# PASSIONLab/ELBA

Measured on AMD Instinct MI355X. Metric: overlap nnz/sec (A·Aᵀ SpGEMM, SharedSeeds semiring, after Prune(numshared<=1)), higher is better.
Workload: dtype u32

## Files before the change

### elba_amd/csrc/capi.hip

```cpp
#include "common.hpp"
#include <new>

using namespace elba;

struct elba_ctx {
    Ctx c;
};

namespace {

template <class F>
int guarded(elba_ctx *ctx, F &&f)
{
    if (!ctx) return ELBA_ERR_INVALID_ARG;
    try {
        ELBA_HIP(hipSetDevice(ctx->c.device));
        f(ctx->c);
        return ELBA_OK;
    } catch (const Error &e) {
        ctx->c.last_error = e.msg;
        return e.code;
    } catch (const std::bad_alloc &) {
        ctx->c.last_error = "host allocation failed";
        return ELBA_ERR_OUT_OF_MEMORY;
// ... 662 lines not shown
                        v->a_csr_format = c.csr_inline ? ELBA_CSR_INLINE : (c.csr_suffix ? ELBA_CSR_DENSE : (c.csr_hints ? ELBA_CSR_HINTS : ELBA_CSR_PLAIN));
                        v->a_csr_pos_mask = c.csr_suffix ? 0xFFFFu : (c.csr_hints ? 0x3FFFFFFFu : 0xFFFFFFFFu);
                        v->a_kmers = c.A_has_kmers ? c.rel_kmers.p : nullptr;
                        v->a_gather_slots = c.use_ell && c.ell_compact ? c.ell_nslots : 0;
                        v->a_slot_kid = c.use_ell && c.ell_compact ? c.ell_slot_kid.p : nullptr; }
        if (c.have_B) { v->Y = c.Y; v->b_rowptr = c.b_rowptr.p; v->b_col = c.b_col.p; v->b_val = c.b_val.p; }
    });
}

int elba_set_option(elba_ctx *ctx, const char *name, int64_t value)
{
    return guarded(ctx, [&](Ctx &c) {
        ELBA_REQUIRE(name, ELBA_ERR_INVALID_ARG, "set_option: null name");
        struct { const char *n; bool *b; } flags[] = {
            {"overlap_cold_calls", &c.cold_calls}, {"no_symmetry", &c.opt.no_symmetry}, {"no_ell", &c.opt.no_ell}, {"no_pay", &c.opt.no_pay}, {"mir32", &c.opt.mir32},
            {"no_hints", &c.opt.no_hints}, {"no_sample", &c.opt.no_sample}, {"no_slab", &c.opt.no_slab}, {"no_ell_compact", &c.opt.no_ell_compact}, {"msd_no_emit8", &c.opt.msd_no_emit8}, {"msd_no_rank", &c.opt.msd_no_rank}, {"msd_rank", &c.opt.msd_rank}, {"csr_pairs_late", &c.opt.csr_pairs_late}, {"no_suffix", &c.opt.no_suffix}, {"ov_generic", &c.opt.ov_generic}, {"no_row_order", &c.opt.no_row_order}, {"no_inline", &c.opt.no_inline}, {"panel_inline", &c.opt.panel_inline}, {"kmer_pairs", &c.opt.kmer_pairs},
            {"kmer_unfused", &c.opt.kmer_unfused}, {"kmer_no_msd", &c.opt.kmer_no_msd}, {"kmer_msd", &c.opt.kmer_msd}, {"csr_pairs", &c.opt.csr_pairs}, {"emit_plain", &c.opt.emit_plain}, {"trace", &c.opt.trace}, {"measure_prep", &c.opt.measure_prep}};
        for (auto &f : flags) if (!strcmp(name, f.n)) { *f.b = value != 0; return; }
        if (!strcmp(name, "kmer_drop")) { ELBA_REQUIRE(value >= 0 && value <= 3, ELBA_ERR_INVALID_ARG, "set_option: kmer_drop is 0..3"); c.opt.kmer_drop = (int)value; }
        else if (!strcmp(name, "dense_up")) { ELBA_REQUIRE(value >= 0 && value <= 3, ELBA_ERR_INVALID_ARG, "set_option: dense_up is 0..3"); c.opt.dense_up = (int)value; }
        else if (!strcmp(name, "dense_wgs")) { ELBA_REQUIRE(value >= 1 && value <= 16, ELBA_ERR_INVALID_ARG, "set_option: dense_wgs is 1..16"); c.opt.dense_wgs = (int)value; }
        else if (!strncmp(name, "tune", 4) && name[4] >= '0' && name[4] <= '7' && name[5] == 0) c.opt.tune[name[4] - '0'] = value;
        else if (!strcmp(name, "msd_small_cap")) c.opt.msd_small_cap = (int)value;
        else if (!strcmp(name, "kmer_batch_instances")) { ELBA_REQUIRE(value >= 0, ELBA_ERR_INVALID_ARG, "set_option: kmer_batch_instances is >= 0"); c.opt.kmer_batch_instances = value; }
        else if (!strcmp(name, "msd_wide_bits")) c.opt.msd_wide_bits = (int)value;
        else if (!strcmp(name, "ell_slot_cap")) c.opt.ell_slot_cap = (int)value;
        else if (!strcmp(name, "slab_pct")) { ELBA_REQUIRE(value >= 1 && value <= 1000, ELBA_ERR_INVALID_ARG, "set_option: slab_pct is 1..1000"); c.opt.slab_pct = (int)value; }
        else if (!strcmp(name, "slab_q16")) { ELBA_REQUIRE(value >= 0 && value < (1ll << 31), ELBA_ERR_INVALID_ARG, "set_option: slab_q16 is 0..2^31"); c.opt.slab_q16 = (int)value; }
        else if (!strcmp(name, "dk")) { ELBA_REQUIRE(value == -1 || value == 0 || value == 1 || value == 2 || value == 4, ELBA_ERR_INVALID_ARG, "set_option: dk is -1 (chosen per matrix), 0, 1, 2 or 4"); c.opt.dk = (int)value; }
        else if (!strcmp(name, "aln_tiers")) { ELBA_REQUIRE(value >= 0, ELBA_ERR_INVALID_ARG, "set_option: aln_tiers is a string of the digits 1, 2, 4, 8"); c.opt.aln_tiers = value; }
        else if (!strcmp(name, "aln_wide_hint")) c.opt.aln_wide_hint = (int)value;
// ... 21 lines not shown

int elba_get_stat(elba_ctx *ctx, const char *name, int64_t *value)
{
    return guarded(ctx, [&](Ctx &c) {
        ELBA_REQUIRE(name && value, ELBA_ERR_INVALID_ARG, "get_stat: null name or value");
        if (!strcmp(name, "overlap_mirror_placed")) *value = c.ov_mir_placed;
        else if (!strcmp(name, "overlap_slab_q16")) *value = (int64_t)c.ov_slab_q16_used;
        else if (!strcmp(name, "kmer_path")) *value = c.kmer_path;
        else if (!strcmp(name, "kmer_passes")) *value = c.kmer_passes;
        else if (!strcmp(name, "kmer_crowded_buckets")) *value = c.kmer_crowded;
        else if (!strcmp(name, "kmer_crowded_small")) *value = c.kmer_crowded_small;
        else if (!strcmp(name, "kmer_largest_pass")) *value = c.kmer_largest_pass;
        else if (!strcmp(name, "kmer_peak_bytes")) *value = c.kmer_peak_bytes;
        else if (!strcmp(name, "kmer_buckets")) *value = c.kmer_buckets;
        else if (!strcmp(name, "overlap_passes")) *value = c.ov_passes;
        else if (!strcmp(name, "overlap_spec")) *value = c.ov_spec;
        else if (!strcmp(name, "overlap_forwarded")) *value = c.ov_forwarded;
        else if (!strcmp(name, "spgemm_prep_us")) *value = c.prep_us;
        else if (!strcmp(name, "emit_us")) *value = c.emit_us;
        else if (!strcmp(name, "triples_path")) *value = c.triples_path;
        else if (!strcmp(name, "padded_columns")) *value = c.have_A && c.use_ell ? 1 : 0;
        else if (!strcmp(name, "gather_slots")) *value = c.have_A && c.use_ell ? c.ell_nslots : 0;
        else if (!strcmp(name, "contig_count")) *value = c.have_contigs ? c.cstats.contigs : 0;
        else if (!strcmp(name, "contig_cycles")) *value = c.have_contigs ? c.cstats.cycles : 0;
        else if (!strcmp(name, "contig_circular")) *value = c.have_contigs ? c.cg_circular : 0;
        else if (!strcmp(name, "contig_singletons")) *value = c.have_contigs ? c.cg_singletons : 0;
        else if (!strcmp(name, "contig_reads")) *value = c.have_contigs ? c.cstats.contig_reads : 0;
        else if (!strcmp(name, "contig_bases")) *value = c.have_contigs ? c.cstats.bases : 0;
        else if (!strcmp(name, "contig_branches")) *value = c.have_contigs ? c.cstats.branches : 0;
        else if (!strcmp(name, "contig_rank_us")) *value = c.have_contigs ? (int64_t)(c.cstats.ms_rank * 1000.0f) : -1;
// ... 150 lines not shown
```

### elba_amd/csrc/common.hpp

```cpp
#pragma once
#include <hip/hip_runtime.h>
#include <cstdint>
#include <cstdio>
#include <cstdlib>
#include <cstring>
#include <mutex>
#include <string>
#include <vector>
#include "../../include/elba_amd.h"

namespace elba {

struct Error {
    int code;
    std::string msg;
};

#define ELBA_HIP(expr)                                                                                   \
    do {                                                                                                 \
        hipError_t e__ = (expr);                                                                         \
        if (e__ != hipSuccess) {                                                                         \
            throw ::elba::Error{e__ == hipErrorOutOfMemory ? ELBA_ERR_OUT_OF_MEMORY : ELBA_ERR_HIP,      \
                                std::string(#expr) + ": " + hipGetErrorString(e__) + " (" + __FILE__ +  \
                                    ":" + std::to_string(__LINE__) + ")"};                               \
// ... 108 lines not shown
    bool no_hints = false;
    bool no_sample = false;
    bool no_ell_compact = false;
    bool no_slab = false;
    bool csr_pairs_late = false;
    bool msd_rank = false;
    bool msd_no_rank = false;
    bool msd_no_emit8 = false;
    int ell_slot_cap = 0;
    int slab_pct = 175;
    int slab_q16 = 0;
    bool panel_inline = false;
    bool no_inline = false;
    bool no_suffix = false;
    bool ov_generic = false;
    bool no_row_order = false;
    bool kmer_pairs = false;
    bool kmer_unfused = false;
    bool kmer_msd = false;
    bool kmer_no_msd = false;
    bool csr_pairs = false;
    bool emit_plain = false;
    bool trace = false;
    bool measure_prep = false;
    int64_t tune[8] = {0, 0, 0, 0, 0, 0, 0, 0};
    int msd_wide_bits = 0;
    int64_t kmer_batch_instances = 0;
    int msd_small_cap = 0;
    int kmer_drop = 0;
    int dense_up = 1;
// ... 128 lines not shown
    DevBuf ov_rowub, ov_rowcnt, ov_rowoff, ov_lists, ov_counters, ov_gtable, ov_sortkeys;
    int64_t ov_tmp_cap = 0;
    bool ov_sort_used[2] = {false, false};
    bool ov_tiers_known = false, ov_tier_used[8] = {false, false, false, false, false, false, false, false};
    int64_t b_cap_entries = 0;
    uint64_t ov_calls = 0;
    uint32_t ov_prior_q16 = 0;
    uint32_t ov_slab_q16 = 0;
    DevBuf ov_slab;
    int64_t ov_slab_cap = 0;
    DevBuf ov_tickrows;
    DevBuf ov_slabpos, ov_slabn;
    bool ov_slab_on = false;
    uint32_t ov_slab_q16_used = 0;
    int64_t ov_mir_placed = 0;
    int64_t ov_spec = 0;
    int64_t ov_passes = 0, ov_forwarded = 0;
    int ov_phase = 0;
    int ov_pend_passes = 1; bool ov_pend_timed = false; float ov_pend_ms[3] = {0, 0, 0};
    std::vector<uint64_t> ov_remote_bounds;
    DevBuf ov_remote;
    int64_t ov_send_slot = 0;
    DevBuf ov_cursors;
    bool own_stream = true;

    EventTimer t_total, t_a, t_b, t_c;
    EventTimer t_emit, t_emit_plain; int64_t prep_us = -1, emit_us = -1;
    struct PinnedHost { void *p = nullptr; size_t cap = 0; void reserve(size_t n) { if (n <= cap) return; if (p) (void)hipHostFree(p); p = nullptr; cap = 0; ELBA_HIP(hipHostMalloc(&p, n, hipHostMallocDefault)); cap = n; } ~PinnedHost() { if (p) (void)hipHostFree(p); } };
    PinnedHost ov_host;
    PhaseMarks<5> ov_marks;
// ... 50 lines not shown
```

### elba_amd/csrc/spgemm.hip

```cpp
#include "common.hpp"
#include <algorithm>
#include <type_traits>

namespace elba {

namespace {

constexpr uint32_t EMPTY = 0xFFFFFFFFu;
constexpr int NUM_LDS_TIERS = 5;
constexpr int NUM_TIERS = NUM_LDS_TIERS + 1;
constexpr int LDS_TBITS0 = 9;
constexpr uint32_t STAGE_CHUNK = 1024;
constexpr uint32_t FIN_WAVE_MAX = 256;
constexpr uint32_t FIN_WAVE2_MAX = 1024;
constexpr uint32_t FIN_LDS_MAX = 4096;

struct alignas(128) OvShard {
    unsigned long long yraw, nnz, ndiag, nupper, fb_claims, fb_ub, products;
    unsigned int maxshared;
    unsigned int tier_done[NUM_TIERS];
};
constexpr int NUM_SHARDS = 64;

struct OvCounters {
// ... 896 lines not shown
    static DeviceOnce attr_once;
    attr_once.run(c.device, [&] {
        const int lds = 160 * 1024;
#define ELBA_ATTR(B, P, D) ELBA_HIP(hipFuncSetAttribute(reinterpret_cast<const void *>(&k_spgemm_direct<B, false, P, D>), hipFuncAttributeMaxDynamicSharedMemorySize, lds))
        ELBA_HIP(hipFuncSetAttribute(reinterpret_cast<const void *>(&k_spgemm_direct<512, false, false, 2, true>), hipFuncAttributeMaxDynamicSharedMemorySize, lds));
        ELBA_HIP(hipFuncSetAttribute(reinterpret_cast<const void *>(&k_spgemm_direct<1024, false, false, 2, true>), hipFuncAttributeMaxDynamicSharedMemorySize, lds));
        ELBA_HIP(hipFuncSetAttribute(reinterpret_cast<const void *>(&k_spgemm_direct<1024, false, false, 2, true, 11>), hipFuncAttributeMaxDynamicSharedMemorySize, lds));
        ELBA_ATTR(512, true, 0); ELBA_ATTR(1024, true, 0); ELBA_ATTR(256, false, 0); ELBA_ATTR(512, false, 0); ELBA_ATTR(1024, false, 0);
        ELBA_ATTR(512, true, 1); ELBA_ATTR(512, true, 2); ELBA_ATTR(512, true, 4); ELBA_ATTR(1024, true, 1); ELBA_ATTR(1024, true, 2); ELBA_ATTR(1024, true, 4);
        ELBA_ATTR(256, false, 1); ELBA_ATTR(256, false, 2); ELBA_ATTR(256, false, 4);
        ELBA_ATTR(512, false, 1); ELBA_ATTR(512, false, 2); ELBA_ATTR(512, false, 4); ELBA_ATTR(1024, false, 1); ELBA_ATTR(1024, false, 2); ELBA_ATTR(1024, false, 4);
#undef ELBA_ATTR
#define ELBA_ATTR(B) ELBA_HIP(hipFuncSetAttribute(reinterpret_cast<const void *>(&k_spgemm_direct<B, false, false, 0, false, 0, true>), hipFuncAttributeMaxDynamicSharedMemorySize, lds))
        ELBA_ATTR(128); ELBA_ATTR(256); ELBA_ATTR(512); ELBA_ATTR(1024);
#undef ELBA_ATTR
    });

    c.ov_host.reserve(sizeof(OvCounters));
    OvCounters &hc = *static_cast<OvCounters *>(c.ov_host.p);
    hc = OvCounters{};
    uint32_t skipped_tiers = 0, skipped_sorts = 0;
    int passes = 0;
    c.ov_passes = 0; c.ov_forwarded = 0; c.ov_spec = 0;
    float ms_sym = 0, ms_num = 0, ms_fin = 0, ms_tot = 0;
    bool was_timed = true;
    for (;;) {
        ++passes;
        const int stride = c.cfg.timing_stride > 1 ? c.cfg.timing_stride : 1;
        const bool timed = passes > 1 || (c.ov_calls++ % (uint64_t)stride) == 0;
        c.ov_tmp.reserve((size_t)c.ov_tmp_cap * sizeof(StageRec));
        p.tmp = c.ov_tmp.as<StageRec>(); p.tmp_cap = (unsigned long long)c.ov_tmp_cap;
        const bool mir16 = c.pos16 && !c.opt.mir32;
        c.ov_rec16 = mir16;
        p.rec16 = mir16 ? 1u : 0u; p.rec = c.ov_tmp.as<uint4>(); p.tick = reinterpret_cast<uint32_t *>(c.ov_tmp.as<char>() + (size_t)c.ov_tmp_cap * 16);
        c.b_cap_entries = half ? 2 * c.ov_tmp_cap : c.ov_tmp_cap;
        c.b_col.reserve((size_t)(c.b_cap_entries + 1) * 4);
        c.b_val.reserve((size_t)(c.b_cap_entries + 1) * sizeof(elba_seed_t));
        if (half) c.ov_mir.reserve((size_t)(c.b_cap_entries + 1) * (mir16 ? 16 : sizeof(StageRec)));
// ... 39 lines not shown
        if (nrows > 0) {
            auto X = [&](int B, bool P) { return (size_t)256 + (size_t)(B / 64) * (P ? 3072 : (pay16 ? 2048 : 2560)); };
            const bool all_tiers = !c.ov_tiers_known || phase == 2;
            skipped_tiers = 0;
            int tmax = NUM_TIERS;
            if (c.opt.tune[4] != 2 && passes == 1) {
                const uint64_t ubm = std::min<uint64_t>((uint64_t)std::max<int64_t>(c.max_row_nnz, 1) * (uint64_t)p.max_col, (uint64_t)p.Mcols);
                const int gmax = ubm <= 1 ? 1 : 64 - __builtin_clzll(2 * ubm - 1);
                tmax = gmax <= LDS_TBITS0 ? 0 : gmax - LDS_TBITS0;
                tmax = std::max(tmax, (int)p.min_tier);
                if (p.suffix) tmax = std::max(tmax, (int)p.dense_up);
            }
#define ELBA_DTIER(t, stmt) do { if ((all_tiers || c.ov_tier_used[t]) && (t) <= tmax) { stmt; } else skipped_tiers |= 1u << (t); } while (0)
#define ELBA_LAUNCH_D(B, G, P, grid, lds, tier, tb, smp)                                                                                  \
    do {                                                                                                                                  \
        if (spec && !(G) && !(P))                                                                                                         \
            hipLaunchKernelGGL((k_spgemm_direct<B, false, false, 0, false, 0, true>), dim3(grid), dim3(B), (lds), s, ov_spec_params(p), (tier), (tb), (smp)); \
        else if (dk == 0) hipLaunchKernelGGL((k_spgemm_direct<B, G, P, 0>), dim3(grid), dim3(B), (lds), s, p, (tier), (tb), (smp));            \
        else if (dk == 1) hipLaunchKernelGGL((k_spgemm_direct<B, G, P, 1>), dim3(grid), dim3(B), (lds), s, p, (tier), (tb), (smp));       \
        else if (dk == 4) hipLaunchKernelGGL((k_spgemm_direct<B, G, P, 4>), dim3(grid), dim3(B), (lds), s, p, (tier), (tb), (smp));       \
        else hipLaunchKernelGGL((k_spgemm_direct<B, G, P, 2>), dim3(grid), dim3(B), (lds), s, p, (tier), (tb), (smp));                    \
    } while (0)
            const int dk = c.opt.dk >= 0 ? c.opt.dk : ((c.csr_inline && c.N > 0 && c.Z < 3 * c.N) ? 0 : 1);
            const bool spec = ov_spec_ok(c, p, pay, dk);
            c.ov_spec = spec ? 1 : 0;
#define ELBA_LAUNCH_S(B, TBC, grid, lds, tier, tb, smp) hipLaunchKernelGGL((k_spgemm_direct<B, false, false, 2, true, TBC>), dim3((tier) == 0 ? cus * c.opt.dense_wgs : (grid)), dim3(B), (size_t)18 * (1u << (tb)) + 256 + (size_t)((B) / 64) * 2368, s, p, (tier), (tb), (smp))
            if (sampling) {
                if (p.suffix) ELBA_LAUNCH_S(1024, 0, cus, (size_t)26 * 4096 + X(1024, true), 3, 12u, 1u);
                else if (pay) ELBA_LAUNCH_D(1024, false, true, cus, (size_t)26 * 4096 + X(1024, true), 3, 12u, 1u);
                else ELBA_LAUNCH_D(1024, false, false, cus, (size_t)18 * 4096 + X(1024, false), 3, 12u, 1u);
                p.use_feedback = 0;
            }
            {
                int nb = (int)((nrows + 255) / 256);
                if (nb > cus * 4) nb = cus * 4;
                hipLaunchKernelGGL(k_classify_direct, dim3(nb), dim3(256), 0, s, p, 0);
            }
            if (p.suffix) {
                ELBA_DTIER(0, ELBA_LAUNCH_S(256, 9, cus * 9, (size_t)26 * 512 + X(128, true), 0, 9u, 0u));
                if (p.dense_up >= 1u) ELBA_DTIER(1, ELBA_LAUNCH_S(512, 10, cus * 4, (size_t)26 * 1024 + X(256, true), 1, 10u, 0u));
// ... 286 lines not shown
```

### elba_amd/csrc/spgemm_direct.hpp

```cpp

enum : uint32_t { D_NEXT = 20, D_FB0 = 16, W_ACC_P = 54 , W_END2 = 56 };
constexpr uint32_t RING = 128;
constexpr uint32_t NOROW = 0xFFFFFFFFu, UNRESOLVED = 0xFFFFFFFEu;

__device__ __forceinline__ uint32_t wave_max_scan(uint32_t v)
{
    int x = (int)v, t;
    t = __builtin_amdgcn_update_dpp(0, x, 0x111 , 0xf, 0xf, false); x = t > x ? t : x;
    t = __builtin_amdgcn_update_dpp(0, x, 0x112 , 0xf, 0xf, false); x = t > x ? t : x;
    t = __builtin_amdgcn_update_dpp(0, x, 0x114 , 0xf, 0xf, false); x = t > x ? t : x;
    t = __builtin_amdgcn_update_dpp(0, x, 0x118 , 0xf, 0xf, false); x = t > x ? t : x;
    t = __builtin_amdgcn_update_dpp(0, x, 0x142 , 0xa, 0xf, false); x = t > x ? t : x;
    t = __builtin_amdgcn_update_dpp(0, x, 0x143 , 0xc, 0xf, false); x = t > x ? t : x;
    return (uint32_t)x;
}

__device__ __forceinline__ uint32_t wave_sum_dpp(uint32_t v)
{
    int x = (int)v;
    x += __builtin_amdgcn_update_dpp(0, x, 0x111 , 0xf, 0xf, false);
    x += __builtin_amdgcn_update_dpp(0, x, 0x112 , 0xf, 0xf, false);
    x += __builtin_amdgcn_update_dpp(0, x, 0x114 , 0xf, 0xf, false);
    x += __builtin_amdgcn_update_dpp(0, x, 0x118 , 0xf, 0xf, false);
    x += __builtin_amdgcn_update_dpp(0, x, 0x142 , 0xa, 0xf, false);
// ... 6 lines not shown
    int x = (int)v;
    x += __builtin_amdgcn_update_dpp(0, x, 0x111 , 0xf, 0xf, false);
    x += __builtin_amdgcn_update_dpp(0, x, 0x112 , 0xf, 0xf, false);
    x += __builtin_amdgcn_update_dpp(0, x, 0x114 , 0xf, 0xf, false);
    x += __builtin_amdgcn_update_dpp(0, x, 0x118 , 0xf, 0xf, false);
    x += __builtin_amdgcn_update_dpp(0, x, 0x142 , 0xa, 0xf, false);
    x += __builtin_amdgcn_update_dpp(0, x, 0x143 , 0xc, 0xf, false);
    return (uint32_t)x;
}

__device__ __forceinline__ bool owns_pair(uint32_t i, uint32_t j, uint32_t row_lo, uint32_t row_hi, bool upper = false)
{
    return j < row_lo || j >= row_hi || (upper ? j > i : ((((i ^ j) & 1u) != 0u) ? j < i : j > i));
}

template <int BLOCK, bool GLOBAL, bool PAY, int DK = 2, bool SUFFIX = false, int TB = 0, bool SPEC = false>
#ifndef ELBA_DENSE_OCC
#define ELBA_DENSE_OCC 8
#endif
__global__ __launch_bounds__(BLOCK, SUFFIX ? ELBA_DENSE_OCC : (DK == 4 ? 1 : 4)) void k_spgemm_direct(std::conditional_t<SPEC, OvSpecParams, OvParams> p, int tier, uint32_t lds_tbits, uint32_t sample)
{
    static_assert(!PAY || !GLOBAL, "payload accumulators: LDS tiers only");
    static_assert(!SPEC || (!GLOBAL && !PAY && !SUFFIX), "the reads path: LDS tiers, 32-bit accumulators carrying posT");
    extern __shared__ __attribute__((aligned(16))) uint32_t smem[];
    uint32_t *misc = GLOBAL ? smem : smem + (size_t)(PAY ? 6 : 4) * (1u << lds_tbits) + ((size_t)1 << lds_tbits) / 2;
    const uint32_t tid = threadIdx.x, lane = tid & 63;
    const uint64_t lt = (1ull << lane) - 1;
    const uint32_t nrows = sample ? p.ctr->sample_count : p.ctr->tier_count[tier];
    if (nrows == 0) return;
    const uint32_t lb = p.lpc_log2, sub = tid & ((1u << lb) - 1u), grp = tid >> lb, EPT = (uint32_t)BLOCK >> lb;
    const uint32_t fbits = p.fbits, fmask = (1u << fbits) - 1u, stride = p.s_stride;
    const bool ell = SPEC || p.a_ell != nullptr;
    const uint32_t hmask = p.hint_mask, pmask = p.pos_mask;
    const uint2 *csr2 = reinterpret_cast<const uint2 *>(p.a_csr);
    const uint32_t slab_q = (p.slab != nullptr && !sample) ? sfirst(p.ctr->slab_q16) : 0u;
    unsigned long long chunk_off = 0;
// ... 126 lines not shown
            tab.keys[s2] = EMPTY; tab.cnt[s2] = 0;
            if (PAY) { tab.vmin[s2] = ~0ull; tab.vmax[s2] = 0ull; } else { tab.smin[s2] = 0xFFFFFFFFu; tab.smax[s2] = 0; }
        };
        const uint32_t DG = GLOBAL ? 0u : dpar;

        bool full = false;
        uint32_t dg = 0, pr = 0;
        uint32_t head = 0, tail = 0;
        const bool pay16 = !PAY && !SUFFIX && !GLOBAL && p.pay16 != 0u;
        uint32_t *qj = misc + 64 + (tid >> 6) * (SUFFIX ? 592u : (PAY ? 768u : (pay16 ? 512u : 640u)));
        uint32_t *qs = qj + RING;
        unsigned long long *qv = reinterpret_cast<unsigned long long *>(qj + RING);
        auto drain = [&](uint32_t n) {
            const uint32_t at = (head + lane) & (RING - 1u);
            const uint32_t j = qj[at];
            if (PAY) { const unsigned long long v = qv[at]; tab.insert_lds64(j, v, v, 1u, lane < n, full); }
            else { const uint32_t sq = qs[at]; tab.insert_lds(j, sq, sq, 1u, lane < n, full); }
            head += n;
        };
        auto slot = [&](uint32_t j, uint32_t posT, uint32_t seq, uint32_t posQ) {
            const uint64_t mv = __ballot(j != EMPTY);
            if (mv == 0) return;
            const uint64_t md = __ballot(j == i);
            pr += (uint32_t)__popcll(mv); dg += (uint32_t)__popcll(md);
            uint64_t mi = mv & ~md;
            if (p.half) mi &= __ballot(owns_pair(i, j, p.half == 2u ? 0u : p.row_lo, p.half == 2u ? 0xFFFFFFFFu : p.row_hi, !PAY && p.suffix != 0u));
            if (mi == 0) return;
            const bool ins = (mi >> lane) & 1ull;
            if (GLOBAL) { if (ins) tab.insert(j, seq, full); return; }
            const uint32_t at = (tail + (uint32_t)__popcll(mi & lt)) & (RING - 1u);
            if (ins) {
                qj[at] = j;
// ... 264 lines not shown
        uint32_t yraw = 0;
        const bool relabel = SUFFIX && p.row_label != nullptr, whole = p.row_lo == 0u && p.row_hi == p.M;
        if (!GLOBAL && T == 4u * (uint32_t)BLOCK) {
            uint32_t jj[4], cc[4], pre[4], tot = 0;
            uint64_t bal[4];
#pragma unroll
            for (int u = 0; u < 4; ++u) { jj[u] = tab.keys[(uint32_t)u * BLOCK + tid]; cc[u] = tab.cnt[(uint32_t)u * BLOCK + tid]; }
            if (SUFFIX && relabel && !whole) {
#pragma unroll
                for (int u = 0; u < 4; ++u) if (jj[u] != EMPTY) jj[u] = p.row_order[jj[u]];
            }
#pragma unroll
            for (int u = 0; u < 4; ++u) {
                const uint32_t j = jj[u];
                if (j != EMPTY) yraw += (p.half == 2u || (p.half && j >= p.row_lo && j < p.row_hi)) ? 2u : 1u;
                bal[u] = __ballot(j != EMPTY && cc[u] >= 2u);
                if (j != EMPTY && cc[u] < 2u) reset_slot((uint32_t)u * BLOCK + tid);
                pre[u] = tot; tot += (uint32_t)__popcll(bal[u]);
            }
            if (tot) {
                uint32_t at = 0;
                if (lane == 0) asm volatile("ds_add_rtn_u32 %0, %1, %2\n\ts_waitcnt lgkmcnt(0)" : "=v"(at) : "v"((uint32_t)(uintptr_t)&misc[3]), "v"(tot) : "memory");
                at = sfirst(at);
#pragma unroll
                for (int u = 0; u < 4; ++u)
                    if ((bal[u] >> lane) & 1ull) list16[at + pre[u] + (uint32_t)__popcll(bal[u] & lt)] = (uint16_t)((uint32_t)u * BLOCK + tid);
            }
        } else
        for (uint32_t b0 = 0; b0 < T; b0 += BLOCK) {
            const uint32_t s0 = b0 + tid;
            bool keep = false;
            if (s0 < T) {
                uint32_t j = tab.ld(tab.keys, s0);
                if (j != EMPTY) {
                    if (SUFFIX && relabel && !whole) j = p.row_order[j];
                    yraw += (p.half == 2u || (p.half && j >= p.row_lo && j < p.row_hi)) ? 2u : 1u; keep = tab.ld(tab.cnt, s0) >= 2;
                    if (!GLOBAL && !keep) reset_slot(s0);
                }
            }
            const uint64_t bal = __ballot(keep);
            if (bal == 0) continue;
            uint32_t at = 0;
            if (lane == 0) at = atomicAdd(&misc[3], (uint32_t)__popcll(bal));
            at = __shfl(at, 0, 64) + (uint32_t)__popcll(bal & lt);
            if (keep) { if (GLOBAL) list[at] = s0; else list16[at] = (uint16_t)s0; }
        }
        yraw = wave_sum_dpp(yraw);
        if (lane == 0 && yraw) lds_add32(&misc[5], yraw);
        if (GLOBAL) __syncthreads(); else lds_barrier();
        ELBA_DSTAMP(4);
        if (tid == 0) {
// ... 29 lines not shown
            const uint32_t ysurv = ysurv_row;
            const uint32_t hasd = dcount_row >= 2 ? 1u : 0u;
            uint32_t nup = 0, mx = 0, nmir = 0;
            bool drew = false;
            auto seed_at = [&](uint32_t a, uint32_t &q, uint32_t &t) {
                const uint2 ce = csr2[rs + (a >> fbits)];
                if (p.inl != 0u && (ce.y >> 31) != 0u) { q = ce.x & 0xFFFFu; t = ce.x >> 16; return; }
                q = ce.x & pmask;
                t = ell ? (uint32_t)p.a_ell[(unsigned long long)ce.y * stride + (a & fmask)] : (uint32_t)p.a_csc[p.a_colptr[ce.y] + (a & fmask)];
            };
            for (uint32_t t = tid; t < ysurv + hasd; t += BLOCK) {
                elba_seed_t v;
                uint32_t j = i;
                if (t < ysurv) {
                    const uint32_t s0 = GLOBAL ? __hip_atomic_load(&list[t], __ATOMIC_RELAXED, __HIP_MEMORY_SCOPE_AGENT) : (uint32_t)list16[t];
                    j = tab.ld(tab.keys, s0); v.numshared = (int32_t)tab.ld(tab.cnt, s0);
                    if (SUFFIX && relabel) j = p.row_order[j];
                    if (PAY) {
                        const uint32_t va = (uint32_t)tab.vmin[s0], vb = (uint32_t)tab.vmax[s0];
                        v.q0 = va >> 16; v.t0 = va & 0xFFFFu; v.q1 = vb >> 16; v.t1 = vb & 0xFFFFu;
                    } else if (pay16) {
                        const uint32_t va = tab.ld(tab.smin, s0), vb = tab.ld(tab.smax, s0);
                        const uint2 ca2 = csr2[rs + ((va >> 16) >> fbits)], cb2 = csr2[rs + ((vb >> 16) >> fbits)];
                        v.q0 = (p.inl != 0u && (ca2.y >> 31) != 0u) ? (ca2.x & 0xFFFFu) : (ca2.x & pmask); v.t0 = va & 0xFFFFu;
                        v.q1 = (p.inl != 0u && (cb2.y >> 31) != 0u) ? (cb2.x & 0xFFFFu) : (cb2.x & pmask); v.t1 = vb & 0xFFFFu;
                    } else {
                        seed_at(tab.ld(tab.smin, s0), v.q0, v.t0);
                        seed_at(tab.ld(tab.smax, s0), v.q1, v.t1);
                    }
                    if (!GLOBAL) reset_slot(s0);
                } else {
// ... 50 lines not shown
        if (*w64(W_MIR)) atomicAdd(&sh->nnz, *w64(W_MIR));
        if (misc[W_MX]) atomicMax(&sh->maxshared, misc[W_MX]);
        unsigned long long fc = *w64(W_FB_C), fu = *w64(W_FB_U);
        if (p.use_feedback && misc[W_FB_N]) { atomicAdd(&p.ctr->fb_claims, fc); atomicAdd(&p.ctr->fb_ub, fu); }
        if (sample && *w64(W_ACC_Y)) atomicAdd(&p.ctr->fb_surv, *w64(W_ACC_Y));
        fc += *w64(W_TOT_C); fu += *w64(W_TOT_U);
        if (fu) { atomicAdd(&sh->fb_claims, fc); atomicAdd(&sh->fb_ub, fu); }
        if (misc[W_ACC_DONE]) {
            atomicAdd(&sh->yraw, *w64(W_ACC_YRAW));
            atomicAdd(&sh->nnz, *w64(W_ACC_Y));
            atomicAdd(&sh->products, *w64(W_ACC_P));
            atomicAdd(&sh->tier_done[tier], misc[W_ACC_DONE]);
            if (misc[W_ACC_NDIAG]) atomicAdd(&sh->ndiag, (unsigned long long)misc[W_ACC_NDIAG]);
        }
    }
}

__global__ __launch_bounds__(256) void k_classify_direct(OvParams p, int mode)
{
    const uint32_t stride = gridDim.x * blockDim.x;
    const uint32_t lane = threadIdx.x & 63;
    const uint64_t lt = (1ull << lane) - 1;
    if (mode == 1) {
        for (uint32_t q = blockIdx.x * blockDim.x + threadIdx.x; q < p.nsample; q += stride) {
            const uint32_t i = p.row_lo + q * p.sstep;
            if (i < p.row_hi && p.a_rowptr[i + 1] != p.a_rowptr[i]) p.sample_list[atomicAdd(&p.ctr->sample_count, 1u)] = i;
        }
        return;
    }
    uint32_t prior_q16 = p.prior_q16;
// ... 67 lines not shown
```

### elba_amd/csrc/spgemm_table.hpp

```cpp
enum : uint32_t {
    W_ACC_YRAW = 32 , W_ACC_Y = 34 , W_ACC_DONE = 36, W_ACC_NDIAG = 37, W_FB_N = 38,
    W_FB_C = 40 , W_FB_U = 42 , W_TOT_C = 44 , W_TOT_U = 46 , W_NUP = 48 , W_MIR = 50 , W_MX = 52, W_END = 54
};
#if defined(ELBA_HMIX_SEL) && ELBA_HMIX_SEL == 1
#define ELBA_HMIX(j) ((j) ^ ((j) >> 5))
#elif defined(ELBA_HMIX_SEL) && ELBA_HMIX_SEL == 2
#define ELBA_HMIX(j) (((j) * 0x85EBCA6Bu) ^ ((j) >> 3))
#elif defined(ELBA_HMIX_SEL) && ELBA_HMIX_SEL == 3
#define ELBA_HMIX(j) ((j) ^ ((j) << 7))
#else
#define ELBA_HMIX(j) (j)
#endif
template <bool GLOBAL>
struct Table {
    uint32_t *keys, *cnt, *smin, *smax, *misc;
    unsigned long long *vmin, *vmax;
    uint32_t tbits, limit;
    __device__ __forceinline__ uint32_t size() const { return 1u << tbits; }
    __device__ __forceinline__ bool abandoned() const { return !GLOBAL && __hip_atomic_load(&misc[10], __ATOMIC_RELAXED, __HIP_MEMORY_SCOPE_WORKGROUP) != 0; }
    __device__ __forceinline__ void insert(uint32_t j, uint32_t s, bool &full) const
    {
        if (full) return;
        const uint32_t mask = size() - 1;
        uint32_t slot = (ELBA_HMIX(j) * 0x9E3779B1u) >> (32 - tbits);
// ... 47 lines not shown
                : [base] "s"(base), [empty] "v"(empty), [j] "v"(j), [mask] "s"(mask), [tb] "s"(tb), [one] "v"(cnt), [s] "v"(s), [smx] "v"(smx)
                : "vcc", "memory");
        }
        if (__ballot(claimed != 0) != 0) {
            uint32_t prev = 0;
            if (claimed) {
                const uint32_t a9 = (uint32_t)(uintptr_t)&misc[9], one = 1u;
                asm volatile("ds_add_rtn_u32 %0, %1, %2\n\ts_waitcnt lgkmcnt(0)" : "=v"(prev) : "v"(a9), "v"(one) : "memory");
            }
            if (__ballot(claimed != 0 && prev >= limit) != 0) {
                misc[10] = 1u;
                full = true;
            }
        }
    }
    __device__ __forceinline__ void insert_lds64(uint32_t j, unsigned long long lo, unsigned long long hi, uint32_t cnt, bool valid, bool &full) const
    {
        if (full) return;
        uint32_t slot = lds_slot(j);
        uint32_t claimed = 0, old, addr = 0;
        unsigned long long save, t;
        const uint32_t base = (uint32_t)(uintptr_t)keys;
        const uint32_t base64 = (uint32_t)(uintptr_t)vmin;
        const uint32_t mask = size() - 1, empty = EMPTY;
        const uint32_t tb = size() * 4, tb8 = size() * 8;
        if (valid) {
            asm volatile(
                "s_mov_b64 %[save], exec\n"
                ".Lprobe%=:\n\t"
                "v_lshl_add_u32 %[addr], %[slot], 2, %[base]\n\t"
                "ds_cmpst_rtn_b32 %[old], %[addr], %[empty], %[j]\n\t"
                "s_waitcnt lgkmcnt(0)\n\t"
                "v_cmp_eq_u32_e64 %[t], %[old], %[empty]\n\t"
                "v_cndmask_b32_e64 %[cl], %[cl], 1, %[t]\n\t"
                "v_cmp_eq_u32_e32 vcc, %[old], %[j]\n\t"
                "s_or_b64 vcc, vcc, %[t]\n\t"
                "s_andn2_b64 exec, exec, vcc\n\t"
                "s_cbranch_execz .Ldone%=\n\t"
                "v_add_u32_e32 %[slot], 1, %[slot]\n\t"
                "v_and_b32_e32 %[slot], %[mask], %[slot]\n\t"
                "s_branch .Lprobe%=\n"
                ".Ldone%=:\n\t"
                "s_mov_b64 exec, %[save]\n\t"
                "v_add_u32_e32 %[old], %[tb], %[addr]\n\t"
                "ds_add_u32 %[old], %[one]\n\t"
                "v_lshl_add_u32 %[old], %[slot], 3, %[base64]\n\t"
                "ds_min_u64 %[old], %[lo]\n\t"
                "v_add_u32_e32 %[old], %[tb8], %[old]\n\t"
                "ds_max_u64 %[old], %[hi]\n"
                : [save] "=&s"(save), [addr] "+v"(addr), [old] "=&v"(old), [t] "=&s"(t), [cl] "+v"(claimed), [slot] "+v"(slot)
                : [base] "s"(base), [base64] "s"(base64), [empty] "v"(empty), [j] "v"(j), [mask] "s"(mask), [tb] "s"(tb), [tb8] "s"(tb8), [one] "v"(cnt), [lo] "v"(lo), [hi] "v"(hi)
                : "vcc", "memory");
        }
        if (__ballot(claimed != 0) != 0) {
            uint32_t prev = 0;
            if (claimed) {
                const uint32_t a9 = (uint32_t)(uintptr_t)&misc[9], one = 1u;
                asm volatile("ds_add_rtn_u32 %0, %1, %2\n\ts_waitcnt lgkmcnt(0)" : "=v"(prev) : "v"(a9), "v"(one) : "memory");
            }
            if (__ballot(claimed != 0 && prev >= limit) != 0) {
                misc[10] = 1u;
                full = true;
            }
        }
    }
    __device__ __forceinline__ uint32_t hit4_lds(const uint32_t (&j)[4], uint32_t s0) const
    {
        typedef __attribute__((address_space(3))) uint32_t lds_u32;
        const lds_u32 *lk = (const lds_u32 *)keys;
        const uint32_t T = size(), tb = T * 4;
        uint32_t slot[4], k[4], m[4];
#pragma unroll
        for (int r = 0; r < 4; ++r) slot[r] = lds_slot(j[r]);
#pragma unroll
        for (int r = 0; r < 4; ++r) {
            k[r] = __hip_atomic_load(&lk[slot[r]], __ATOMIC_RELAXED, __HIP_MEMORY_SCOPE_WORKGROUP);
            m[r] = __hip_atomic_load(&lk[slot[r] + 2u * T], __ATOMIC_RELAXED, __HIP_MEMORY_SCOPE_WORKGROUP);
        }
        uint32_t miss = 0;
        const uint32_t base = (uint32_t)(uintptr_t)keys, one = 1u;
// ... 110 lines not shown
```

Measured before the change: 16.93 billion.

## Aggregate hash-table claim counting per wavefront and skip count add on claim

```diff
diff --git a/elba_amd/csrc/capi.hip b/elba_amd/csrc/capi.hip
--- a/elba_amd/csrc/capi.hip
+++ b/elba_amd/csrc/capi.hip
@@ -700,7 +700,7 @@
         ELBA_REQUIRE(name, ELBA_ERR_INVALID_ARG, "set_option: null name");
         struct { const char *n; bool *b; } flags[] = {
             {"overlap_cold_calls", &c.cold_calls}, {"no_symmetry", &c.opt.no_symmetry}, {"no_ell", &c.opt.no_ell}, {"no_pay", &c.opt.no_pay}, {"mir32", &c.opt.mir32},
-            {"no_hints", &c.opt.no_hints}, {"no_sample", &c.opt.no_sample}, {"no_slab", &c.opt.no_slab}, {"no_ell_compact", &c.opt.no_ell_compact}, {"msd_no_emit8", &c.opt.msd_no_emit8}, {"msd_no_rank", &c.opt.msd_no_rank}, {"msd_rank", &c.opt.msd_rank}, {"csr_pairs_late", &c.opt.csr_pairs_late}, {"no_suffix", &c.opt.no_suffix}, {"ov_generic", &c.opt.ov_generic}, {"no_row_order", &c.opt.no_row_order}, {"no_inline", &c.opt.no_inline}, {"panel_inline", &c.opt.panel_inline}, {"kmer_pairs", &c.opt.kmer_pairs},
+            {"no_hints", &c.opt.no_hints}, {"no_sample", &c.opt.no_sample}, {"no_slab", &c.opt.no_slab}, {"no_ell_compact", &c.opt.no_ell_compact}, {"msd_no_emit8", &c.opt.msd_no_emit8}, {"msd_no_rank", &c.opt.msd_no_rank}, {"msd_rank", &c.opt.msd_rank}, {"csr_pairs_late", &c.opt.csr_pairs_late}, {"no_suffix", &c.opt.no_suffix}, {"ov_generic", &c.opt.ov_generic}, {"ov_claim_legacy", &c.opt.ov_claim_legacy}, {"no_row_order", &c.opt.no_row_order}, {"no_inline", &c.opt.no_inline}, {"panel_inline", &c.opt.panel_inline}, {"kmer_pairs", &c.opt.kmer_pairs},
             {"kmer_unfused", &c.opt.kmer_unfused}, {"kmer_no_msd", &c.opt.kmer_no_msd}, {"kmer_msd", &c.opt.kmer_msd}, {"csr_pairs", &c.opt.csr_pairs}, {"emit_plain", &c.opt.emit_plain}, {"trace", &c.opt.trace}, {"measure_prep", &c.opt.measure_prep}};
         for (auto &f : flags) if (!strcmp(name, f.n)) { *f.b = value != 0; return; }
         if (!strcmp(name, "kmer_drop")) { ELBA_REQUIRE(value >= 0 && value <= 3, ELBA_ERR_INVALID_ARG, "set_option: kmer_drop is 0..3"); c.opt.kmer_drop = (int)value; }
@@ -752,6 +752,7 @@
         else if (!strcmp(name, "kmer_peak_bytes")) *value = c.kmer_peak_bytes;
         else if (!strcmp(name, "kmer_buckets")) *value = c.kmer_buckets;
         else if (!strcmp(name, "overlap_passes")) *value = c.ov_passes;
+        else if (!strcmp(name, "overlap_claim_insert")) *value = c.ov_claim_insert;
         else if (!strcmp(name, "overlap_spec")) *value = c.ov_spec;
         else if (!strcmp(name, "overlap_forwarded")) *value = c.ov_forwarded;
         else if (!strcmp(name, "spgemm_prep_us")) *value = c.prep_us;
diff --git a/elba_amd/csrc/common.hpp b/elba_amd/csrc/common.hpp
--- a/elba_amd/csrc/common.hpp
+++ b/elba_amd/csrc/common.hpp
@@ -146,6 +146,7 @@
     bool no_inline = false;
     bool no_suffix = false;
     bool ov_generic = false;
+    bool ov_claim_legacy = false;
     bool no_row_order = false;
     bool kmer_pairs = false;
     bool kmer_unfused = false;
@@ -304,6 +305,7 @@
     bool ov_slab_on = false;
     uint32_t ov_slab_q16_used = 0;
     int64_t ov_mir_placed = 0;
+    int64_t ov_claim_insert = 1;
     int64_t ov_spec = 0;
     int64_t ov_passes = 0, ov_forwarded = 0;
     int ov_phase = 0;
diff --git a/elba_amd/csrc/spgemm.hip b/elba_amd/csrc/spgemm.hip
--- a/elba_amd/csrc/spgemm.hip
+++ b/elba_amd/csrc/spgemm.hip
@@ -934,6 +934,9 @@
 #define ELBA_ATTR(B) ELBA_HIP(hipFuncSetAttribute(reinterpret_cast<const void *>(&k_spgemm_direct<B, false, false, 0, false, 0, true>), hipFuncAttributeMaxDynamicSharedMemorySize, lds))
         ELBA_ATTR(128); ELBA_ATTR(256); ELBA_ATTR(512); ELBA_ATTR(1024);
 #undef ELBA_ATTR
+#define ELBA_ATTR(B) ELBA_HIP(hipFuncSetAttribute(reinterpret_cast<const void *>(&k_spgemm_direct_claim0<B>), hipFuncAttributeMaxDynamicSharedMemorySize, lds))
+        ELBA_ATTR(128); ELBA_ATTR(256); ELBA_ATTR(512); ELBA_ATTR(1024);
+#undef ELBA_ATTR
     });
 
     c.ov_host.reserve(sizeof(OvCounters));
@@ -941,7 +944,7 @@
     hc = OvCounters{};
     uint32_t skipped_tiers = 0, skipped_sorts = 0;
     int passes = 0;
-    c.ov_passes = 0; c.ov_forwarded = 0; c.ov_spec = 0;
+    c.ov_passes = 0; c.ov_forwarded = 0; c.ov_spec = 0; c.ov_claim_insert = 1;
     float ms_sym = 0, ms_num = 0, ms_fin = 0, ms_tot = 0;
     bool was_timed = true;
     for (;;) {
@@ -1011,7 +1014,9 @@
 #define ELBA_DTIER(t, stmt) do { if ((all_tiers || c.ov_tier_used[t]) && (t) <= tmax) { stmt; } else skipped_tiers |= 1u << (t); } while (0)
 #define ELBA_LAUNCH_D(B, G, P, grid, lds, tier, tb, smp)                                                                                  \
     do {                                                                                                                                  \
-        if (spec && !(G) && !(P))                                                                                                         \
+        if (spec && !(G) && !(P) && c.opt.ov_claim_legacy)                                                                                \
+            hipLaunchKernelGGL((k_spgemm_direct_claim0<B>), dim3(grid), dim3(B), (lds), s, ov_spec_params(p), (tier), (tb), (smp));       \
+        else if (spec && !(G) && !(P))                                                                                                    \
             hipLaunchKernelGGL((k_spgemm_direct<B, false, false, 0, false, 0, true>), dim3(grid), dim3(B), (lds), s, ov_spec_params(p), (tier), (tb), (smp)); \
         else if (dk == 0) hipLaunchKernelGGL((k_spgemm_direct<B, G, P, 0>), dim3(grid), dim3(B), (lds), s, p, (tier), (tb), (smp));            \
         else if (dk == 1) hipLaunchKernelGGL((k_spgemm_direct<B, G, P, 1>), dim3(grid), dim3(B), (lds), s, p, (tier), (tb), (smp));       \
@@ -1021,6 +1026,7 @@
             const int dk = c.opt.dk >= 0 ? c.opt.dk : ((c.csr_inline && c.N > 0 && c.Z < 3 * c.N) ? 0 : 1);
             const bool spec = ov_spec_ok(c, p, pay, dk);
             c.ov_spec = spec ? 1 : 0;
+            c.ov_claim_insert = spec ? (c.opt.ov_claim_legacy ? 0 : 2) : 1;
 #define ELBA_LAUNCH_S(B, TBC, grid, lds, tier, tb, smp) hipLaunchKernelGGL((k_spgemm_direct<B, false, false, 2, true, TBC>), dim3((tier) == 0 ? cus * c.opt.dense_wgs : (grid)), dim3(B), (size_t)18 * (1u << (tb)) + 256 + (size_t)((B) / 64) * 2368, s, p, (tier), (tb), (smp))
             if (sampling) {
                 if (p.suffix) ELBA_LAUNCH_S(1024, 0, cus, (size_t)26 * 4096 + X(1024, true), 3, 12u, 1u);
diff --git a/elba_amd/csrc/spgemm_direct.hpp b/elba_amd/csrc/spgemm_direct.hpp
--- a/elba_amd/csrc/spgemm_direct.hpp
+++ b/elba_amd/csrc/spgemm_direct.hpp
@@ -44,12 +44,12 @@
     return j < row_lo || j >= row_hi || (upper ? j > i : ((((i ^ j) & 1u) != 0u) ? j < i : j > i));
 }
 
-template <int BLOCK, bool GLOBAL, bool PAY, int DK = 2, bool SUFFIX = false, int TB = 0, bool SPEC = false>
-#ifndef ELBA_DENSE_OCC
-#define ELBA_DENSE_OCC 8
-#endif
-__global__ __launch_bounds__(BLOCK, SUFFIX ? ELBA_DENSE_OCC : (DK == 4 ? 1 : 4)) void k_spgemm_direct(std::conditional_t<SPEC, OvSpecParams, OvParams> p, int tier, uint32_t lds_tbits, uint32_t sample)
+template <int BLOCK, bool GLOBAL, bool PAY, int DK, bool SUFFIX, int TB, bool SPEC, int INS>
+__device__ __forceinline__ void spgemm_direct_rows(std::conditional_t<SPEC, OvSpecParams, OvParams> p, int tier, uint32_t lds_tbits, uint32_t sample)
 {
+    static_assert(INS != 0 || (SPEC && !PAY), "the insert of rounds 1-6: kept for the reads path's A/B only");
+    static_assert(INS == 0 || INS == 1 || (INS == 2 && SPEC), "count - 1 in the count words: the reads path only");
+    constexpr uint32_t CKEEP = INS == 2 ? 1u : 2u, CBIAS = INS == 2 ? 1u : 0u;
     static_assert(!PAY || !GLOBAL, "payload accumulators: LDS tiers only");
     static_assert(!SPEC || (!GLOBAL && !PAY && !SUFFIX), "the reads path: LDS tiers, 32-bit accumulators carrying posT");
     extern __shared__ __attribute__((aligned(16))) uint32_t smem[];
@@ -206,8 +206,8 @@
         auto drain = [&](uint32_t n) {
             const uint32_t at = (head + lane) & (RING - 1u);
             const uint32_t j = qj[at];
-            if (PAY) { const unsigned long long v = qv[at]; tab.insert_lds64(j, v, v, 1u, lane < n, full); }
-            else { const uint32_t sq = qs[at]; tab.insert_lds(j, sq, sq, 1u, lane < n, full); }
+            if (PAY) { const unsigned long long v = qv[at]; tab.template insert_lds64_agg<false>(j, v, v, 1u, lane < n, full); }
+            else { const uint32_t sq = qs[at]; if (INS == 0) tab.insert_lds(j, sq, sq, 1u, lane < n, full); else tab.template insert_lds_agg<INS == 2>(j, sq, sq, 1u, lane < n, full); }
             head += n;
         };
         auto slot = [&](uint32_t j, uint32_t posT, uint32_t seq, uint32_t posQ) {
@@ -502,8 +502,8 @@
             for (int u = 0; u < 4; ++u) {
                 const uint32_t j = jj[u];
                 if (j != EMPTY) yraw += (p.half == 2u || (p.half && j >= p.row_lo && j < p.row_hi)) ? 2u : 1u;
-                bal[u] = __ballot(j != EMPTY && cc[u] >= 2u);
-                if (j != EMPTY && cc[u] < 2u) reset_slot((uint32_t)u * BLOCK + tid);
+                bal[u] = __ballot(j != EMPTY && cc[u] >= CKEEP);
+                if (j != EMPTY && cc[u] < CKEEP) reset_slot((uint32_t)u * BLOCK + tid);
                 pre[u] = tot; tot += (uint32_t)__popcll(bal[u]);
             }
             if (tot) {
@@ -522,7 +522,7 @@
                 uint32_t j = tab.ld(tab.keys, s0);
                 if (j != EMPTY) {
                     if (SUFFIX && relabel && !whole) j = p.row_order[j];
-                    yraw += (p.half == 2u || (p.half && j >= p.row_lo && j < p.row_hi)) ? 2u : 1u; keep = tab.ld(tab.cnt, s0) >= 2;
+                    yraw += (p.half == 2u || (p.half && j >= p.row_lo && j < p.row_hi)) ? 2u : 1u; keep = tab.ld(tab.cnt, s0) >= CKEEP;
                     if (!GLOBAL && !keep) reset_slot(s0);
                 }
             }
@@ -582,7 +582,7 @@
                 uint32_t j = i;
                 if (t < ysurv) {
                     const uint32_t s0 = GLOBAL ? __hip_atomic_load(&list[t], __ATOMIC_RELAXED, __HIP_MEMORY_SCOPE_AGENT) : (uint32_t)list16[t];
-                    j = tab.ld(tab.keys, s0); v.numshared = (int32_t)tab.ld(tab.cnt, s0);
+                    j = tab.ld(tab.keys, s0); v.numshared = (int32_t)(tab.ld(tab.cnt, s0) + CBIAS);
                     if (SUFFIX && relabel) j = p.row_order[j];
                     if (PAY) {
                         const uint32_t va = (uint32_t)tab.vmin[s0], vb = (uint32_t)tab.vmax[s0];
@@ -663,6 +663,20 @@
             if (misc[W_ACC_NDIAG]) atomicAdd(&sh->ndiag, (unsigned long long)misc[W_ACC_NDIAG]);
         }
     }
+}
+
+template <int BLOCK, bool GLOBAL, bool PAY, int DK = 2, bool SUFFIX = false, int TB = 0, bool SPEC = false>
+#ifndef ELBA_DENSE_OCC
+#define ELBA_DENSE_OCC 8
+#endif
+__global__ __launch_bounds__(BLOCK, SUFFIX ? ELBA_DENSE_OCC : (DK == 4 ? 1 : 4)) void k_spgemm_direct(std::conditional_t<SPEC, OvSpecParams, OvParams> p, int tier, uint32_t lds_tbits, uint32_t sample)
+{
+    spgemm_direct_rows<BLOCK, GLOBAL, PAY, DK, SUFFIX, TB, SPEC, SPEC ? 2 : 1>(p, tier, lds_tbits, sample);
+}
+template <int BLOCK>
+__global__ __launch_bounds__(BLOCK, 4) void k_spgemm_direct_claim0(OvSpecParams p, int tier, uint32_t lds_tbits, uint32_t sample)
+{
+    spgemm_direct_rows<BLOCK, false, false, 0, false, 0, true, 0>(p, tier, lds_tbits, sample);
 }
 
 __global__ __launch_bounds__(256) void k_classify_direct(OvParams p, int mode)
diff --git a/elba_amd/csrc/spgemm_table.hpp b/elba_amd/csrc/spgemm_table.hpp
--- a/elba_amd/csrc/spgemm_table.hpp
+++ b/elba_amd/csrc/spgemm_table.hpp
@@ -85,56 +85,116 @@
             }
         }
     }
-    __device__ __forceinline__ void insert_lds64(uint32_t j, unsigned long long lo, unsigned long long hi, uint32_t cnt, bool valid, bool &full) const
+    template <bool CM1>
+    __device__ __forceinline__ void insert_lds_agg(uint32_t j, uint32_t s, uint32_t smx, uint32_t cnt, bool valid, bool &full) const
     {
         if (full) return;
         uint32_t slot = lds_slot(j);
-        uint32_t claimed = 0, old, addr = 0;
-        unsigned long long save, t;
-        const uint32_t base = (uint32_t)(uintptr_t)keys;
+        uint32_t old, addr = 0, prev, n, k;
+        unsigned long long save, t, cm;
+        const unsigned long long vm = __ballot(valid);
+        const uint32_t base = (uint32_t)(uintptr_t)keys, a9 = (uint32_t)(uintptr_t)&misc[9];
+        const uint32_t mask = size() - 1, empty = EMPTY;
+        const uint32_t tb = size() * 4;
+#define ELBA_AGG_PROBE                                                                                                                    \
+                "s_mov_b64 %[save], exec\n\t"                                                                                             \
+                "s_and_b64 exec, exec, %[vm]\n\t"                                                                                         \
+                "s_mov_b64 %[cm], 0\n\t"                                                                                                  \
+                "s_mov_b32 %[prev], 0\n"                                                                                                  \
+                ".Lprobe%=:\n\t"                                                                                                          \
+                "v_lshl_add_u32 %[addr], %[slot], 2, %[base]\n\t"                                                                         \
+                "ds_cmpst_rtn_b32 %[old], %[addr], %[empty], %[j]\n\t"                                                                    \
+                "s_waitcnt lgkmcnt(0)\n\t"                                                                                                \
+                "v_cmp_eq_u32_e64 %[t], %[old], %[empty]\n\t"                                                                             \
+                "s_or_b64 %[cm], %[cm], %[t]\n\t"                                                                                         \
+                "v_cmp_eq_u32_e32 vcc, %[old], %[j]\n\t"                                                                                  \
+                "s_or_b64 vcc, vcc, %[t]\n\t"                                                                                             \
+                "s_andn2_b64 exec, exec, vcc\n\t"                                                                                         \
+                "s_cbranch_execz .Ldone%=\n\t"                                                                                            \
+                "v_add_u32_e32 %[slot], 1, %[slot]\n\t"                                                                                   \
+                "v_and_b32_e32 %[slot], %[mask], %[slot]\n\t"                                                                             \
+                "s_branch .Lprobe%=\n"                                                                                                    \
+                ".Ldone%=:\n\t"                                                                                                           \
+                "s_and_b64 exec, %[save], %[vm]\n\t"
+#define ELBA_AGG_CLAIMS                                                                                                                   \
+                "s_bcnt1_i32_b64 %[n], %[cm]\n\t"                                                                                         \
+                "s_cbranch_scc0 .Lnone%=\n\t"                                                                                             \
+                "s_ff1_i32_b64 %[k], %[save]\n\t"                                                                                         \
+                "s_lshl_b64 exec, 1, %[k]\n\t"                                                                                            \
+                "v_mov_b32_e32 %[old], %[n]\n\t"                                                                                          \
+                "v_mov_b32_e32 %[addr], %[a9]\n\t"                                                                                        \
+                "ds_add_rtn_u32 %[old], %[addr], %[old]\n\t"                                                                              \
+                "s_waitcnt lgkmcnt(0)\n\t"                                                                                                \
+                "v_readfirstlane_b32 %[prev], %[old]\n"                                                                                   \
+                ".Lnone%=:\n\t"                                                                                                           \
+                "s_mov_b64 exec, %[save]\n"
+        if (CM1)
+            asm volatile(
+                ELBA_AGG_PROBE
+                "v_add_u32_e32 %[old], %[tb], %[addr]\n\t"
+                "s_andn2_b64 exec, exec, %[cm]\n\t"
+                "ds_add_u32 %[old], %[one]\n\t"
+                "s_and_b64 exec, %[save], %[vm]\n\t"
+                "v_add_u32_e32 %[old], %[tb], %[old]\n\t"
+                "ds_min_u32 %[old], %[s]\n\t"
+                "v_add_u32_e32 %[old], %[tb], %[old]\n\t"
+                "ds_max_u32 %[old], %[smx]\n\t"
+                ELBA_AGG_CLAIMS
+                : [save] "=&s"(save), [addr] "+v"(addr), [old] "=&v"(old), [t] "=&s"(t), [cm] "=&s"(cm), [prev] "=&s"(prev), [n] "=&s"(n), [k] "=&s"(k), [slot] "+v"(slot)
+                : [vm] "s"(vm), [base] "s"(base), [a9] "s"(a9), [empty] "v"(empty), [j] "v"(j), [mask] "s"(mask), [tb] "s"(tb), [one] "v"(cnt), [s] "v"(s), [smx] "v"(smx)
+                : "vcc", "scc", "memory");
+        else
+            asm volatile(
+                ELBA_AGG_PROBE
+                "v_add_u32_e32 %[old], %[tb], %[addr]\n\t"
+                "ds_add_u32 %[old], %[one]\n\t"
+                "v_add_u32_e32 %[old], %[tb], %[old]\n\t"
+                "ds_min_u32 %[old], %[s]\n\t"
+                "v_add_u32_e32 %[old], %[tb], %[old]\n\t"
+                "ds_max_u32 %[old], %[smx]\n\t"
+                ELBA_AGG_CLAIMS
+                : [save] "=&s"(save), [addr] "+v"(addr), [old] "=&v"(old), [t] "=&s"(t), [cm] "=&s"(cm), [prev] "=&s"(prev), [n] "=&s"(n), [k] "=&s"(k), [slot] "+v"(slot)
+                : [vm] "s"(vm), [base] "s"(base), [a9] "s"(a9), [empty] "v"(empty), [j] "v"(j), [mask] "s"(mask), [tb] "s"(tb), [one] "v"(cnt), [s] "v"(s), [smx] "v"(smx)
+                : "vcc", "scc", "memory");
+        if (CM1 && cnt > 1u && ((cm >> __builtin_amdgcn_mbcnt_hi(~0u, __builtin_amdgcn_mbcnt_lo(~0u, 0u))) & 1ull) != 0)
+            asm volatile("ds_add_u32 %0, %1" : : "v"(base + tb + (slot << 2)), "v"(cnt - 1u) : "memory");
+        if (prev + n > limit) {
+            misc[10] = 1u;
+            full = true;
+        }
+    }
+    template <bool CM1>
+    __device__ __forceinline__ void insert_lds64_agg(uint32_t j, unsigned long long lo, unsigned long long hi, uint32_t cnt, bool valid, bool &full) const
+    {
+        static_assert(!CM1, "64-bit accumulators: the general kernel, whole counts");
+        if (full) return;
+        uint32_t slot = lds_slot(j);
+        uint32_t old, addr = 0, prev, n, k;
+        unsigned long long save, t, cm;
+        const unsigned long long vm = __ballot(valid);
+        const uint32_t base = (uint32_t)(uintptr_t)keys, a9 = (uint32_t)(uintptr_t)&misc[9];
         const uint32_t base64 = (uint32_t)(uintptr_t)vmin;
         const uint32_t mask = size() - 1, empty = EMPTY;
         const uint32_t tb = size() * 4, tb8 = size() * 8;
-        if (valid) {
-            asm volatile(
-                "s_mov_b64 %[save], exec\n"
-                ".Lprobe%=:\n\t"
-                "v_lshl_add_u32 %[addr], %[slot], 2, %[base]\n\t"
-                "ds_cmpst_rtn_b32 %[old], %[addr], %[empty], %[j]\n\t"
-                "s_waitcnt lgkmcnt(0)\n\t"
-                "v_cmp_eq_u32_e64 %[t], %[old], %[empty]\n\t"
-                "v_cndmask_b32_e64 %[cl], %[cl], 1, %[t]\n\t"
-                "v_cmp_eq_u32_e32 vcc, %[old], %[j]\n\t"
-                "s_or_b64 vcc, vcc, %[t]\n\t"
-                "s_andn2_b64 exec, exec, vcc\n\t"
-                "s_cbranch_execz .Ldone%=\n\t"
-                "v_add_u32_e32 %[slot], 1, %[slot]\n\t"
-                "v_and_b32_e32 %[slot], %[mask], %[slot]\n\t"
-                "s_branch .Lprobe%=\n"
-                ".Ldone%=:\n\t"
-                "s_mov_b64 exec, %[save]\n\t"
-                "v_add_u32_e32 %[old], %[tb], %[addr]\n\t"
-                "ds_add_u32 %[old], %[one]\n\t"
-                "v_lshl_add_u32 %[old], %[slot], 3, %[base64]\n\t"
-                "ds_min_u64 %[old], %[lo]\n\t"
-                "v_add_u32_e32 %[old], %[tb8], %[old]\n\t"
-                "ds_max_u64 %[old], %[hi]\n"
-                : [save] "=&s"(save), [addr] "+v"(addr), [old] "=&v"(old), [t] "=&s"(t), [cl] "+v"(claimed), [slot] "+v"(slot)
-                : [base] "s"(base), [base64] "s"(base64), [empty] "v"(empty), [j] "v"(j), [mask] "s"(mask), [tb] "s"(tb), [tb8] "s"(tb8), [one] "v"(cnt), [lo] "v"(lo), [hi] "v"(hi)
-                : "vcc", "memory");
-        }
-        if (__ballot(claimed != 0) != 0) {
-            uint32_t prev = 0;
-            if (claimed) {
-                const uint32_t a9 = (uint32_t)(uintptr_t)&misc[9], one = 1u;
-                asm volatile("ds_add_rtn_u32 %0, %1, %2\n\ts_waitcnt lgkmcnt(0)" : "=v"(prev) : "v"(a9), "v"(one) : "memory");
-            }
-            if (__ballot(claimed != 0 && prev >= limit) != 0) {
-                misc[10] = 1u;
-                full = true;
-            }
-        }
-    }
+        asm volatile(
+            ELBA_AGG_PROBE
+            "v_add_u32_e32 %[old], %[tb], %[addr]\n\t"
+            "ds_add_u32 %[old], %[one]\n\t"
+            "v_lshl_add_u32 %[old], %[slot], 3, %[base64]\n\t"
+            "ds_min_u64 %[old], %[lo]\n\t"
+            "v_add_u32_e32 %[old], %[tb8], %[old]\n\t"
+            "ds_max_u64 %[old], %[hi]\n\t"
+            ELBA_AGG_CLAIMS
+            : [save] "=&s"(save), [addr] "+v"(addr), [old] "=&v"(old), [t] "=&s"(t), [cm] "=&s"(cm), [prev] "=&s"(prev), [n] "=&s"(n), [k] "=&s"(k), [slot] "+v"(slot)
+            : [vm] "s"(vm), [base] "s"(base), [base64] "s"(base64), [a9] "s"(a9), [empty] "v"(empty), [j] "v"(j), [mask] "s"(mask), [tb] "s"(tb), [tb8] "s"(tb8), [one] "v"(cnt), [lo] "v"(lo), [hi] "v"(hi)
+            : "vcc", "scc", "memory");
+        if (prev + n > limit) {
+            misc[10] = 1u;
+            full = true;
+        }
+    }
+#undef ELBA_AGG_PROBE
+#undef ELBA_AGG_CLAIMS
     __device__ __forceinline__ uint32_t hit4_lds(const uint32_t (&j)[4], uint32_t s0) const
     {
         typedef __attribute__((address_space(3))) uint32_t lds_u32;
```

Measured after the change: 17.07 billion, median of 2. No clear change (+0.8%).
